# hjr37/diff-gaussian-rasterization

Hardware: AMD Instinct MI355X
Metric: Mviews/sec fwd+bwd @1080p, 500k Gaussians (higher is better)
Workload: dtype f32

## Files before the change

diff-gaussian-rasterization_amd/csrc/render_common.h:

```cpp
#pragma once
#include "dgr_common.h"
#include "kernels.h"
#include "wave_reduce.h"
#include "exact_math.h"

namespace dgr {

__device__ __forceinline__ uint4 blend_slot(const uint4* __restrict__ sched, const uint2* __restrict__ ranges,
                                            const uint32_t* __restrict__ sched_flag, int tiles, bool* overflowed = nullptr,
                                            bool* quadrant_lists = nullptr) {
    const int flag = __builtin_amdgcn_readfirstlane((int)*sched_flag);
    if (overflowed) *overflowed = (flag & 2) != 0;
    if (quadrant_lists) *quadrant_lists = (flag & 4) != 0;
    if (flag & 1) return sched[blockIdx.x];
    const int tile = xcd_contiguous((int)blockIdx.x, tiles);
    const uint2 r = ranges[tile];
    return make_uint4((uint32_t)tile, r.x, r.y, 0u);
}

__device__ __forceinline__ bool wave_any(bool p) { return __builtin_amdgcn_ballot_w64(p) != 0ull; }

namespace {

constexpr float LOG2E = 1.4426950408889634f, LN2 = 0.6931471805599453f;
constexpr float ALPHA_MIN = 15.0f / 255.0f;

enum { ALPHA_REF = 0, ALPHA_FAST = 1, ALPHA_GLIBC = 2 };
template <int AM>
struct AlphaPath {
    static constexpr bool LOG2 = (AM == ALPHA_FAST);
    static constexpr float PSCALE = LOG2 ? LOG2E : 1.0f;
    static constexpr float PUNSCALE = LOG2 ? LN2 : 1.0f;
    static constexpr bool TABLE = (AM == ALPHA_GLIBC);
};
template <int AM, bool UNTESTED_ARG = false>
__device__ __forceinline__ float alpha_raw(float o, float p2, const uint64_t* tab) {
    if (AM == ALPHA_FAST) return o * __builtin_amdgcn_exp2f(p2);
    if (AM == ALPHA_GLIBC) return o * exp_glibc<UNTESTED_ARG>(p2, tab);
    return o * exp_p32<UNTESTED_ARG>(p2);
}
template <int AM>
__device__ __forceinline__ float t_div(float T, float om, float& inv) {
    if (AM == ALPHA_FAST) { inv = __builtin_amdgcn_rcpf(om); return T * inv; }
    return div_ref(T, om, inv);
}

template <int NB, typename LIST_T = unsigned short, int NLISTS = 4, bool KEEP_ID = true>
struct StagedT {
    typedef LIST_T list_t;
    static constexpr bool HAS_ID = KEEP_ID;
    static constexpr int SLOTS = NB;
    static constexpr int SENTINEL = NB;
    static constexpr int LIST_LD = NB + 8;
    float4 rec[2 * (NB + 1)];
    float4 rgbd[NB + 1];
    uint32_t id[KEEP_ID ? NB : 1];
    LIST_T list[NLISTS][LIST_LD];
    int cnt4[4][NLISTS];
};
using Staged = StagedT<DGR_TILE_PIX>;

template <bool HALF_CODES>
__device__ __forceinline__ unsigned reach_code(const float4& q0, const float4& q1, float l2, float tile_x0, float tile_y0);

template <int AM, bool HALF_CODES = false, class S>
__device__ __forceinline__ unsigned stage_one(S& s, int slot, uint32_t gid, const float4* __restrict__ rec,
                                              float tile_x0, float tile_y0) {
    const float4 q0 = rec[DGR_REC_STRIDE * (size_t)gid + 0];
    const float4 q1 = rec[DGR_REC_STRIDE * (size_t)gid + 1];
    const float4 q2 = rec[DGR_REC_STRIDE * (size_t)gid + 2];
    const float o = q0.w;
    const float l2 = __log2f(o * (255.0f / 15.0f));
    constexpr float PSCALE = AlphaPath<AM>::PSCALE;
    float lthr = (o > 0.f) ? (-l2 * (AlphaPath<AM>::LOG2 ? 1.0f : LN2) - 1.0e-4f) : 3.0e38f;
    float zword = __int_as_float(slot);
    if (HALF_CODES) {
        lthr = fmaxf(lthr, -3.0e38f);
        lthr = __int_as_float(((__float_as_int(lthr) + 0xFF) & ~0xFF) | slot);
        zword = 0.f;
    }
    s.rec[2 * slot] = make_float4(q0.x, q0.y, -0.5f * PSCALE * q1.x, -0.5f * PSCALE * q1.z);
    s.rec[2 * slot + 1] = make_float4(-PSCALE * q1.y, o, zword, lthr);
    s.rgbd[slot] = make_float4(q2.x, q2.y, q2.z, q0.z);
    if (S::HAS_ID) s.id[slot] = gid;
    return reach_code<HALF_CODES>(q0, q1, l2, tile_x0, tile_y0);
}
template <bool HALF_CODES>
__device__ __forceinline__ unsigned reach_code(const float4& q0, const float4& q1, float l2, float tile_x0, float tile_y0) {
    const float tau = 2.0f * 0.6931471805599453f * l2;
    const float det = q1.x * q1.z - q1.y * q1.y;
    if (!(tau > 0.0f)) return 0u;
    if (!(det > 0.0f && q1.x > 0.0f && q1.z > 0.0f)) return HALF_CODES ? 0xFFu : 0xFu;
    const float k = tau * __builtin_amdgcn_rcpf(det);
    const float hx = __builtin_amdgcn_sqrtf(k * q1.z) * 1.001f + 0.05f, hy = __builtin_amdgcn_sqrtf(k * q1.x) * 1.001f + 0.05f;
    const float gx = q0.x - tile_x0, gy = q0.y - tile_y0;
    const bool xl = (gx + hx >= 0.0f) && (gx - hx <= 7.0f), xr = (gx + hx >= 8.0f) && (gx - hx <= 15.0f);
    if (HALF_CODES) {
        const float lo = gy - hy, hi = gy + hy;
        const unsigned xm = (xl ? 0x33u : 0u) | (xr ? 0xCCu : 0u);
        const unsigned ym = ((hi >= 0.0f) && (lo <= 3.0f) ? 0x05u : 0u) | ((hi >= 4.0f) && (lo <= 7.0f) ? 0x0Au : 0u) |
                            ((hi >= 8.0f) && (lo <= 11.0f) ? 0x50u : 0u) | ((hi >= 12.0f) && (lo <= 15.0f) ? 0xA0u : 0u);
        return xm & ym;
    }
    const bool yt = (gy + hy >= 0.0f) && (gy - hy <= 7.0f), yb = (gy + hy >= 8.0f) && (gy - hy <= 15.0f);
    return (xl && yt ? 1u : 0u) | (xr && yt ? 2u : 0u) | (xl && yb ? 4u : 0u) | (xr && yb ? 8u : 0u);
}

constexpr int TAG_SHIFT = DGR_TAG_SHIFT;
constexpr uint32_t ID_MASK = DGR_ID_MASK;
enum { TAGS_BYTES_QUADRANT = 1, TAGS_BYTES_HALVES = 2 };

__device__ __forceinline__ uint8_t* half_tags(const uint32_t* point_list, const uint32_t* sched_flag) {
    return carve_binning(reinterpret_cast<char*>(const_cast<uint32_t*>(point_list)), (size_t)sched_flag[-1]).pair_cov;
}
__device__ __forceinline__ uint32_t spread4(uint32_t c) { return (c & 1u) | ((c & 2u) << 1) | ((c & 4u) << 2) | ((c & 8u) << 3); }
__device__ __forceinline__ uint32_t fold8(uint32_t t) {
    t = (t | (t >> 1)) & 0x55u;
    return (t & 1u) | ((t >> 1) & 2u) | ((t >> 2) & 4u) | ((t >> 3) & 8u);
}

__device__ __forceinline__ uint32_t pack4(uint32_t w) { return (w & 1u) | ((w >> 7) & 2u) | ((w >> 14) & 4u) | ((w >> 21) & 8u); }
__device__ __forceinline__ uint32_t tag_byte(uint32_t up, uint32_t lo) { return spread4(pack4(up)) | (spread4(pack4(lo)) << 1); }

template <int AM, int TAGS, class S>
__device__ __forceinline__ unsigned stage_tagged(S& s, int slot, uint32_t entry, const float4* __restrict__ rec,
                                                 const uint8_t* __restrict__ tag8) {
    constexpr float PSCALE = AlphaPath<AM>::PSCALE;
    unsigned code = (unsigned)*tag8;
    if (code == 0u) return 0u;
    if (TAGS == TAGS_BYTES_QUADRANT) code = fold8(code);
    const uint32_t gid = entry & ID_MASK;
    const float4 q0 = rec[DGR_REC_STRIDE * (size_t)gid + 0];
    const float4 q1 = rec[DGR_REC_STRIDE * (size_t)gid + 1];
    const float4 q2 = rec[DGR_REC_STRIDE * (size_t)gid + 2];
    s.rec[2 * slot] = make_float4(q0.x, q0.y, -0.5f * PSCALE * q1.x, -0.5f * PSCALE * q1.z);
    s.rec[2 * slot + 1] = make_float4(-PSCALE * q1.y, q0.w, __int_as_float(slot * 4), __int_as_float(slot * 16));
    s.rgbd[slot] = make_float4(q2.x, q2.y, q2.z, q0.z);
    s.id[slot] = gid;
    return code;
}

__device__ __forceinline__ int lanes_below(unsigned long long m) {
    return (int)__builtin_amdgcn_mbcnt_hi((unsigned)(m >> 32), __builtin_amdgcn_mbcnt_lo((unsigned)m, 0u));
}

template <class S>
__device__ __forceinline__ int build_lists(S& s, unsigned code, int tid, int wave, int lane) {
    typedef typename S::list_t LT;
    unsigned long long bal[4];
#pragma unroll
    for (int w = 0; w < 4; w++) {
        bal[w] = __ballot((code >> w) & 1u);
        if (lane == 0) s.cnt4[wave][w] = __popcll(bal[w]);
    }
    __syncthreads();
#pragma unroll
    for (int w = 0; w < 4; w++) {
        if ((code >> w) & 1u) {
            int base = 0;
            for (int sw = 0; sw < wave; sw++) base += s.cnt4[sw][w];
            s.list[w][base + lanes_below(bal[w])] = (LT)(tid * 32);
        }
    }
    const int n = __builtin_amdgcn_readfirstlane(s.cnt4[0][wave] + s.cnt4[1][wave] + s.cnt4[2][wave] + s.cnt4[3][wave]);
    __syncthreads();
    if (lane < 4) s.list[wave][n + lane] = (LT)(S::SENTINEL * 32);
    return n;
}

template <class S>
__device__ __forceinline__ int build_half_lists(S& s, unsigned code, int tid, int wave, int lane) {
    typedef typename S::list_t LT;
    unsigned long long bal[8];
#pragma unroll
    for (int l = 0; l < 8; l++) {
        bal[l] = __ballot((code >> l) & 1u);
        if (lane == 0) s.cnt4[wave][l] = __popcll(bal[l]);
    }
    __syncthreads();
    int before = 0, all = 0;
    if (lane < 8) {
#pragma unroll
        for (int sw = 0; sw < 4; sw++) {
            const int c = s.cnt4[sw][lane];
            before += sw < wave ? c : 0;
            all += c;
        }
    }
#pragma unroll
    for (int l = 0; l < 8; l++) {
        const int base = __builtin_amdgcn_readlane(before, l);
        if ((code >> l) & 1u) s.list[l][base + lanes_below(bal[l])] = (LT)(tid * 32);
    }
    const int l0 = 2 * wave;
    const int n0 = __builtin_amdgcn_readlane(all, l0), n1 = __builtin_amdgcn_readlane(all, l0 + 1);
    __syncthreads();
    const int n = max(n0, n1);
    for (int i = n0 + lane; i < n + 4; i += 64) s.list[l0][i] = (LT)(S::SENTINEL * 32);
    for (int i = n1 + lane; i < n + 4; i += 64) s.list[l0 + 1][i] = (LT)(S::SENTINEL * 32);
    return n;
}

template <class S>
__device__ __forceinline__ int build_paired_lists(S& s, unsigned code8, int tid, int wave, int lane, unsigned long long (&split)[2]) {
    typedef typename S::list_t LT;
    static_assert(sizeof(LT) == 4 && S::SLOTS <= 128, "paired lists: 32-bit entries, at most two ranks per lane");
    unsigned long long bal[4];
#pragma unroll
    for (int w = 0; w < 4; w++) {
        bal[w] = __ballot(((code8 >> (2 * w)) & 3u) != 0u);
        if (lane == 0) s.cnt4[wave][w] = __popcll(bal[w]);
    }
    __syncthreads();
    int before = 0, all = 0;
    if (lane < 4) {
#pragma unroll
        for (int sw = 0; sw < 4; sw++) {
            const int c = s.cnt4[sw][lane];
            before += sw < wave ? c : 0;
            all += c;
        }
    }
#pragma unroll
    for (int w = 0; w < 4; w++) {
        const unsigned t = (code8 >> (2 * w)) & 3u;
        const int base = __builtin_amdgcn_readlane(before, w);
        if (t != 0u) s.list[2 * w][base + lanes_below(bal[w])] = (LT)(tid * 32) | t;
    }
    const int n = __builtin_amdgcn_readlane(all, wave);
    __syncthreads();
    LT* const LU = s.list[2 * wave];
    LT* const LL = s.list[2 * wave + 1];
    if (n <= 64) {
        const bool have = lane < n;
        const unsigned e0 = have ? LU[lane] : 0u;
        const int t0 = (int)(e0 & 3u);
        const int tm1 = __builtin_amdgcn_update_dpp(0, t0, 0x138, 0xf, 0xf, true);
        const int tm2 = __builtin_amdgcn_update_dpp(0, tm1, 0x138, 0xf, 0xf, true);
        const int tp1 = __builtin_amdgcn_update_dpp(0, t0, 0x130, 0xf, 0xf, true);
        const int tp2 = __builtin_amdgcn_update_dpp(0, tp1, 0x130, 0xf, 0xf, true);
        const bool odd = (lane & 1) != 0;
        const bool a_self = odd ? (tm1 * t0 == 2) : (t0 * tp1 == 2);
        const bool a_side = odd ? (tp1 * tp2 == 2) : (tm2 * tm1 == 2);
        const bool p2 = !a_self && !a_side && (odd ? (t0 * tp1 == 2) : (tm1 * t0 == 2));
        const bool first = odd ? p2 : a_self, second = odd ? a_self : p2;
        const unsigned long long keep = __ballot(have && !second);
        const int steps = __popcll(keep);
        if (have) {
            const int st = lanes_below(keep) - (second ? 1 : 0);
            const LT o = e0 & ~3u;
            if (first || second) {
                (t0 == 1 ? LU : LL)[st] = o;
            } else {
                LU[st] = o;
                LL[st] = o;
            }
        }
        if (lane < 4) {
            LU[steps + lane] = (LT)(S::SENTINEL * 32);
            LL[steps + lane] = (LT)(S::SENTINEL * 32);
        }
        split[0] = __ballot(lane < steps && LU[lane] != LL[lane]);
        split[1] = 0ull;
        return steps;
    }
    const LT ea = lane < n ? LU[lane] : 0u, eb = lane + 64 < n ? LU[lane + 64] : 0u;
    if (lane < n) { LU[lane] = ea & ~3u; LL[lane] = ea & ~3u; }
    if (lane + 64 < n) { LU[lane + 64] = eb & ~3u; LL[lane + 64] = eb & ~3u; }
    if (lane < 4) {
        LU[n + lane] = (LT)(S::SENTINEL * 32);
        LL[n + lane] = (LT)(S::SENTINEL * 32);
    }
    split[0] = split[1] = 0ull;
    return n;
}

typedef float f2 __attribute__((ext_vector_type(2)));

template <int AM>
__device__ __forceinline__ float pair_p2(const float4& q0, const float4& q1, f2 pxy, f2& dxy) {
    const f2 g = {q0.x, q0.y}, ac = {q0.z, q0.w};
    dxy = g - pxy;
    if (AM == ALPHA_FAST) {
        const f2 m = ac * dxy;
        const float t = __builtin_fmaf(q1.x, dxy.y, m.x);
        return __builtin_fmaf(dxy.x, t, m.y * dxy.y);
    } else {
#pragma clang fp contract(off)
        const f2 m = (ac * dxy) * dxy;
        const float B = (q1.x * dxy.x) * dxy.y;
        return (m.x + m.y) + B;
    }
}

template <class S>
__device__ __forceinline__ void load2(const S& s, int wave, int k, float4 (&q0)[2], float4 (&q1)[2]) {
    typedef typename S::list_t LT;
    unsigned off[2];
    if (sizeof(LT) == 4) {
        const uint2 pk = *reinterpret_cast<const uint2*>(&s.list[wave][k]);
        off[0] = pk.x;
        off[1] = pk.y;
    } else {
        const unsigned pk = *reinterpret_cast<const unsigned*>(&s.list[wave][k]);
        off[0] = pk & 0xffffu;
        off[1] = pk >> 16;
    }
    const char* base = reinterpret_cast<const char*>(s.rec);
#pragma unroll
    for (int u = 0; u < 2; u++) {
        q0[u] = *reinterpret_cast<const float4*>(base + off[u]);
        q1[u] = *reinterpret_cast<const float4*>(base + off[u] + 16);
    }
}


template <bool TAGGED = false, class S>
__device__ __forceinline__ void write_sentinel(S& s) {
    constexpr int NB = S::SLOTS;
    s.rec[2 * NB] = make_float4(0.f, 0.f, 0.f, 0.f);
    s.rec[2 * NB + 1] = make_float4(0.f, 0.f, __int_as_float(TAGGED ? NB * 4 : NB), TAGGED ? __int_as_float(NB * 16) : 3.0e38f);
    s.rgbd[NB] = make_float4(0.f, 0.f, 0.f, 0.f);
}

constexpr int NACC = DGR_ACC_STRIDE;
constexpr int ACC_LD = DGR_TILE_PIX + 1;

template <int NCOMP, int LD = ACC_LD>
__device__ __forceinline__ void flush_acc(const float* lds_acc, const uint32_t* ids, int cnt, float* global_acc, int tid) {
    const int comp = tid & 15;
    if (comp < NCOMP) {
        for (int r = tid >> 4; r < cnt; r += 16) {
            const float v = lds_acc[comp * LD + r];
            if (v != 0.f) atomicAdd(global_acc + (size_t)ids[r] * DGR_ACC_STRIDE + comp, v);
        }
    }
}

}
}
```

diff-gaussian-rasterization_amd/csrc/render_light.hip:

```cpp
#include "render_common.h"

namespace dgr {
namespace {

constexpr int FWD_UNROLL = 2;

template <bool HALVES>
struct StagedFwd {
    typedef StagedT<DGR_TILE_PIX, unsigned short, HALVES ? 8 : 4, !HALVES> staged_t;
    staged_t f;
    float unc[DGR_TILE_PIX];
    uint32_t cnt[DGR_TILE_PIX];
    uint32_t hit[DGR_TILE_PIX];
    uint64_t exptab[32];
};


template <class SF>
__device__ __forceinline__ void flush_slot(const SF& sf, const RenderFwdLightArgs& a, uint8_t* tag8, uint32_t pos0, int tid, bool staged) {
    if (!staged) return;
    uint32_t t8;
    if constexpr (!SF::staged_t::HAS_ID) {
        t8 = tag_byte(sf.hit[tid], __float_as_uint(sf.f.rec[2 * tid + 1].z));
    } else {
        t8 = spread4(pack4(sf.hit[tid])) * 3u;
    }
    tag8[pos0 + tid] = (uint8_t)t8;
    if (sf.cnt[tid] != 0u) {
        uint32_t gid;
        if constexpr (SF::staged_t::HAS_ID) gid = sf.f.id[tid];
        else gid = a.point_list[pos0 + tid];
        atomicAdd(&a.gau_uncertainty[gid], sf.unc[tid]);
        atomicAdd(&a.gau_related_pixels[gid], (int)sf.cnt[tid]);
    }
}

template <int AM, bool HALVES>
__device__ __forceinline__ void render_fwd_light_body(const RenderFwdLightArgs& a, StagedFwd<HALVES>& sf, const uint4 slot, const bool overflowed) {
    typename StagedFwd<HALVES>::staged_t& s = sf.f;
    const int tile = (int)slot.x;
    const int tx = tile % a.grid_x, ty = tile / a.grid_x;
    const int tid = threadIdx.x, wave = tid >> 6, lane = tid & 63;
    const int px = tx * DGR_BLOCK_X + (wave & 1) * 8 + (lane & 7);
    const int py = ty * DGR_BLOCK_Y + (wave >> 1) * 8 + (lane >> 3);
    const bool inside = px < a.W && py < a.H;
    const uint32_t pix_id = (uint32_t)a.W * (uint32_t)py + (uint32_t)px;
    const f2 pxy = {(float)px, (float)py};
    const float tile_x0 = (float)(tx * DGR_BLOCK_X), tile_y0 = (float)(ty * DGR_BLOCK_Y);
    const int my_list = HALVES ? 2 * wave + (lane >> 5) : wave;
    uint8_t* const tag8 = half_tags(a.point_list, a.sched_flag);
    unsigned char* const mark_base = (HALVES && lane >= 32) ? reinterpret_cast<unsigned char*>(&s.rec[1].z) + wave
                                                             : reinterpret_cast<unsigned char*>(sf.hit) + wave;
    const int mark_stride = (HALVES && lane >= 32) ? 32 : 4;

    const uint2 range = make_uint2(slot.y, slot.z);
    const int total = (int)(range.y - range.x);

    float T = 1.0f, C0 = 0.f, C1 = 0.f, C2 = 0.f, weight = 0.f, Dd = 0.f, D_median = 0.f;
    uint32_t last_contributor = 0;
    float ub = inside ? 0.f : -__builtin_inff();
    const float gt_px = inside ? a.gt_depth[pix_id] : 0.f;
    if (tid == 0) write_sentinel(s);
    if (AlphaPath<AM>::TABLE) exp_ref_table_fill(sf.exptab, tid);
    bool have_flush = false;
    int last_base = 0;

    for (int base = 0; base < total; base += DGR_TILE_PIX) {
        if (__syncthreads_and(ub < 0.f)) break;
        last_base = base;
        if (have_flush) flush_slot(sf, a, tag8, range.x + base - DGR_TILE_PIX, tid, true);
        sf.unc[tid] = 0.f;
        sf.cnt[tid] = 0u;
        sf.hit[tid] = 0u;
        have_flush = true;
        const int cnt = min(DGR_TILE_PIX, total - base);
        unsigned code = 0;
        if (tid < cnt) code = stage_one<AM, HALVES>(s, tid, a.point_list[range.x + base + tid], a.rec, tile_x0, tile_y0);
        const int n = HALVES ? build_half_lists(s, code, tid, wave, lane) : build_lists(s, code, tid, wave, lane);

        for (int k = 0; k < n; k += FWD_UNROLL) {
            float4 q0[FWD_UNROLL], q1[FWD_UNROLL];
            load2(s, my_list, k, q0, q1);
#pragma unroll
            for (int u = 0; u < FWD_UNROLL; u++) {
                f2 dxy;
                const float p2 = pair_p2<AM>(q0[u], q1[u], pxy, dxy);
                if ((p2 <= ub) & (p2 >= q1[u].w)) {
                  const float alpha = fminf(0.99f, alpha_raw<AM>(q1[u].y, p2, sf.exptab));
                  if (alpha >= ALPHA_MIN) {
#pragma clang fp contract(off)
                    const float test_T = T * (1.0f - alpha);
                    if (test_T < 0.0001f) {
                        ub = -__builtin_inff();
                    } else {
                        const int j = HALVES ? (__float_as_int(q1[u].w) & 0xFF) : __float_as_int(q1[u].z);
                        const float4 cd = s.rgbd[j];
                        mark_base[j * mark_stride] = 1;
                        const float w = alpha * T;
                        C0 = __builtin_fmaf(cd.x, w, C0); C1 = __builtin_fmaf(cd.y, w, C1); C2 = __builtin_fmaf(cd.z, w, C2);
                        weight = weight + w;
                        Dd = __builtin_fmaf(cd.w, w, Dd);
                        if (T > 0.5f && test_T < 0.5f) {
                            D_median = cd.w;
                            const float e = cd.w - gt_px;
                            atomicAdd(&sf.unc[j], e * e * w);
                            atomicAdd(&sf.cnt[j], 1u);
                        }
                        T = test_T;
                        last_contributor = (uint32_t)(base + j + 1);
                    }
                  }
                }
            }
            if (!wave_any(ub >= 0.f)) break;
        }
    }
    __syncthreads();
    if (have_flush) flush_slot(sf, a, tag8, range.x + last_base, tid, tid < total - last_base);
    for (int p = (have_flush ? last_base + DGR_TILE_PIX : 0) + tid; p < total; p += DGR_TILE_PIX) tag8[range.x + p] = 0;

    if (overflowed) {
        C0 = C1 = C2 = weight = Dd = D_median = __builtin_nanf("");
    }
    if (inside) {
        const uint32_t N = (uint32_t)a.W * (uint32_t)a.H;
        a.n_contrib[pix_id] = last_contributor;
        a.out_color[pix_id] = C0 + T * a.bg[0];
        a.out_color[N + pix_id] = C1 + T * a.bg[1];
        a.out_color[2 * N + pix_id] = C2 + T * a.bg[2];
        a.out_alpha[pix_id] = weight;
        a.out_depth[pix_id] = Dd;
        a.out_median[pix_id] = D_median;
        a.out_depth_var[pix_id] = 0.0f;
    }
}

template <int AM>
__global__ void __launch_bounds__(256, 8) render_fwd_light_kernel(RenderFwdLightArgs a) {
    __shared__ union { StagedFwd<true> h; StagedFwd<false> q; } sf;
    if (a.rep.host && blockIdx.x == 0 && threadIdx.x == 0) report_status(a.rep, a.status);
    bool overflowed, quadrant_lists;
    const uint4 slot = blend_slot(a.sched, a.ranges, a.sched_flag, a.grid_x * a.grid_y, &overflowed, &quadrant_lists);
    if (quadrant_lists) render_fwd_light_body<AM, false>(a, sf.q, slot, overflowed);
    else render_fwd_light_body<AM, true>(a, sf.h, slot, overflowed);
}

constexpr int NACC_LIGHT = 14;

template <bool DET, bool HALVES = false, bool ABS = false>
struct StagedBwd {
    static constexpr int NB = DET ? 64 : 128;
    static constexpr int LD = NB + 1;
    static constexpr int PLANE = NACC_LIGHT * LD;
    static constexpr int NACC = ABS ? NACC_LIGHT + 2 : NACC_LIGHT;
    typedef StagedT<NB, uint32_t, HALVES ? 8 : 4> staged_t;
    staged_t f;
    float acc[(DET ? 4 : 1) * PLANE + (ABS ? 2 * LD : 0)];
    uint32_t inst[DET ? NB : 1];
    int max_last;
    uint64_t exptab[32];
};

template <int AM, bool DO_MAP, bool DO_POSE, bool DET, bool LEAN, bool HALVES, bool ABS = false>
__device__ __forceinline__ void render_bwd_light_body(const RenderBwdLightArgs& a, StagedBwd<DET, HALVES, ABS>& sb, const uint4 slot,
                                                      float* __restrict__ abs_out = nullptr) {
    static_assert(!HALVES || !DET, "half-wave / paired lists: not with the deterministic kernel's planes (LDS)");
    static_assert(!ABS || (DO_MAP && !DET), "absgrad: the mapping backward, not the deterministic kernel");
    constexpr bool PAIRED = HALVES && DO_MAP;
    typedef StagedBwd<DET, HALVES, ABS> SB;
    constexpr int BWD_NB = SB::NB, BWD_LD = SB::LD;
    typename SB::staged_t& s = sb.f;
    const int tile = (int)slot.x;
    const int tx = tile % a.grid_x, ty = tile / a.grid_x;
    const int tid = threadIdx.x, wave = tid >> 6, lane = tid & 63;
    const int px = tx * DGR_BLOCK_X + (wave & 1) * 8 + (lane & 7);
    const int py = ty * DGR_BLOCK_Y + (wave >> 1) * 8 + (lane >> 3);
    const bool inside = px < a.W && py < a.H;
    const uint32_t pix_id = (uint32_t)a.W * (uint32_t)py + (uint32_t)px;
    const uint32_t N = (uint32_t)a.W * (uint32_t)a.H;
    const float pxf = (float)px, pyf = (float)py;
    const f2 pxy = {pxf, pyf};

    const uint2 range = make_uint2(slot.y, slot.z);
    const int last_contributor = inside ? (int)a.n_contrib[pix_id] : 0;

    if (tid == 0) {
        sb.max_last = 0;
        write_sentinel<true>(s);
    }
    if (AlphaPath<AM>::TABLE) exp_ref_table_fill(sb.exptab, tid);
    __syncthreads();
    {
        int v = last_contributor;
#pragma unroll
        for (int off = 32; off > 0; off >>= 1) v = max(v, __shfl_xor(v, off, 64));
        if (lane == 0) atomicMax(&sb.max_last, v);
    }
    __syncthreads();
    const int total = min((int)(range.y - range.x), sb.max_last);
    if (total <= 0) return;

    const float T_final = inside ? (1.0f - a.alphas[pix_id]) : 0.f;
    float T = T_final;
    float dpix0 = 0.f, dpix1 = 0.f, dpix2 = 0.f, dpix_depth = 0.f, dpix_median = 0.f, dpix_var = 0.f, gt_px = 0.f;
    if (inside) {
        dpix0 = __builtin_nontemporal_load(a.dL_dpix + pix_id);
        dpix1 = __builtin_nontemporal_load(a.dL_dpix + N + pix_id);
        dpix2 = __builtin_nontemporal_load(a.dL_dpix + 2 * N + pix_id);
        dpix_depth = __builtin_nontemporal_load(a.dL_dpix_depth + pix_id);
        if (!LEAN) {
            if (a.dL_dpix_median) dpix_median = __builtin_nontemporal_load(a.dL_dpix_median + pix_id);
            if (a.dL_dpix_var) dpix_var = __builtin_nontemporal_load(a.dL_dpix_var + pix_id);
            gt_px = __builtin_nontemporal_load(a.gt_depth + pix_id);
        }
    }
    const float bg_term = -T_final * (a.bg[0] * dpix0 + a.bg[1] * dpix1 + a.bg[2] * dpix2);
    const float ddelx_dx = 0.5f * a.W, ddely_dy = 0.5f * a.H;
    float S = 0.f;
    float mid_thr = 0.5f;
    int my_comp;
    if (DO_MAP) {
        const int c = (lane >= 48) ? 12 : wave_reduce12d_comp(lane);
        my_comp = ((lane & 3) != 0 || c > 11) ? -1 : (c == 10 ? (DO_POSE ? 13 : 10) : c == 11 ? (DO_POSE ? 10 : -1) : c);
    } else if (HALVES) {
        const int c = half_reduce3_comp(lane);
        my_comp = c == 0 ? 4 : c == 1 ? 5 : c == 2 ? 13 : -1;
    } else {
        const int c = wave_reduce4_comp(lane);
        my_comp = ((lane & 15) == 0 && c < 3) ? (c == 0 ? 4 : c == 1 ? 5 : 13) : -1;
    }
    const int my_list = HALVES ? 2 * wave + (lane >> 5) : wave;
    const uint8_t* const tag8 = half_tags(a.point_list, a.sched_flag);

    float* const my_acc = sb.acc + (DET ? wave * SB::PLANE : 0) + (my_comp >= 0 ? my_comp : 0) * BWD_LD;

    for (int hi = total; hi > 0; hi -= BWD_NB) {
        const int lo = max(0, hi - BWD_NB);
        const int cnt = hi - lo;
        __syncthreads();
        unsigned code = 0;
        if (tid < cnt) code = stage_tagged<AM, HALVES ? TAGS_BYTES_HALVES : TAGS_BYTES_QUADRANT>(s, tid, a.point_list[range.x + lo + tid], a.rec, tag8 + (range.x + lo + tid));
        if (!DET) {
#pragma unroll
            for (int k = 0; k < SB::NACC; k++)
                if (BWD_NB == DGR_TILE_PIX || tid < BWD_NB) sb.acc[k * BWD_LD + tid] = 0.f;
        }
        unsigned long long split[2] = {0ull, 0ull};
        const int n = PAIRED   ? build_paired_lists(s, code, tid, wave, lane, split)
                      : HALVES ? build_half_lists(s, code, tid, wave, lane)
                               : build_lists(s, code, tid, wave, lane);
        const int rel_last4 = 4 * (last_contributor - lo);

        constexpr int U = PAIRED ? 1 : 2;
        for (int k = ((n + U - 1) / U) * U - U; k >= 0; k -= U) {
            float4 q0[2], q1[2];
            if (U == 2) {
                load2(s, my_list, k, q0, q1);
            } else {
                const unsigned off = s.list[my_list][k];
                q0[0] = *reinterpret_cast<const float4*>(reinterpret_cast<const char*>(s.rec) + off);
                q1[0] = *reinterpret_cast<const float4*>(reinterpret_cast<const char*>(s.rec) + off + 16);
            }
#pragma unroll
            for (int u = U - 1; u >= 0; u--) {
                f2 dxy;
                const float p2 = pair_p2<AM>(q0[u], q1[u], pxy, dxy);
                const float dx = dxy.x, dy = dxy.y;
                const int j4 = __float_as_int(q1[u].z);
                const float oG = alpha_raw<AM, true>(q1[u].y, p2, sb.exptab);
                const bool valid = (j4 < rel_last4) & (p2 <= 0.0f) & !(oG < ALPHA_MIN);
                const float oGm = valid ? oG : 0.f;
                const float alpha = fminf(0.99f, oGm);
                const float4 cd = *reinterpret_cast<const float4*>(reinterpret_cast<const char*>(s.rgbd) + __float_as_int(q1[u].w));
                const float om = 1.f - alpha;
                float inv;
                T = t_div<AM>(T, om, inv);
                const float w = alpha * T;
                const float e = cd.w - gt_px;
                const float X = LEAN ? cd.x * dpix0 + cd.y * dpix1 + cd.z * dpix2 + cd.w * dpix_depth
                                     : cd.x * dpix0 + cd.y * dpix1 + cd.z * dpix2 + cd.w * dpix_depth + (e * e) * dpix_var;
                const float dL_dalpha = (X - S) * T + bg_term * inv;
                S = alpha * X + om * S;
                const float qq = oGm * dL_dalpha;
                const float qdx = qq * dx, qdy = qq * dy;
                const float wd = w * dpix_depth;
                float tot;
                if (DO_MAP) {
                    float gmed = 0.f;
                    if (!LEAN) {
                        const bool fire = valid & (T > mid_thr);
                        gmed = fire ? dpix_median : 0.f;
                        mid_thr = fire ? __builtin_inff() : mid_thr;
                    }
                    float g[12];
                    g[0] = w * dpix0;
                    g[1] = w * dpix1;
                    g[2] = w * dpix2;
                    g[3] = LEAN ? wd : wd + 2.f * ((dpix_var * w) * e);
                    g[4] = qdx;
                    g[5] = qdy;
                    g[6] = qdx * dx;
                    g[7] = qdx * dy;
                    g[8] = qdy * dy;
                    g[9] = qq;
                    g[10] = DO_POSE ? wd : gmed;
                    g[11] = DO_POSE ? gmed : 0.f;
                    if (ABS) {
                        constexpr float UN = AlphaPath<AM>::PUNSCALE;
                        const float ca = q0[u].z * (-2.f * UN), cb = q1[u].x * (-UN), cc = q0[u].w * (-2.f * UN);
                        const float h = half_reduce3(fabsf(ca * qdx + cb * qdy), fabsf(cc * qdy + cb * qdx), 0.f);
                        const int c = half_reduce3_comp(lane);
                        if (c == 0 || c == 1)
                            atomicAdd(reinterpret_cast<float*>(reinterpret_cast<char*>(sb.acc) + j4 + (NACC_LIGHT + c) * (BWD_LD * 4)), h);
                    }
                    if (PAIRED) {
                        float u0, u1;
                        wave_reduce12d_head(g, u0, u1);
                        const int st = k + u;
                        if ((split[st >> 6] >> (st & 63)) & 1ull) {
                            const float r0 = quad_sum(u0), r1 = quad_sum(u1);
                            auto comp_of = [](int slot) { return slot < 10 ? slot : slot == 10 ? (DO_POSE ? 13 : 10) : (DO_POSE ? 10 : -1); };
                            const int s1 = wave_reduce12d_half_slot1(lane);
                            const int c0 = (lane & 3) == 0 ? comp_of(wave_reduce12d_half_slot0(lane)) : -1;
                            const int c1 = ((lane & 3) == 0 && s1 >= 0) ? comp_of(s1) : -1;
                            char* const col = reinterpret_cast<char*>(sb.acc) + j4;
                            if (c0 >= 0) atomicAdd(reinterpret_cast<float*>(col + c0 * (BWD_LD * 4)), r0);
                            if (c1 >= 0) atomicAdd(reinterpret_cast<float*>(col + c1 * (BWD_LD * 4)), r1);
                            continue;
                        }
                        tot = wave_reduce12d_tail(u0, u1);
                    } else {
                        tot = wave_reduce12d(g);
                    }
                } else if (HALVES) {
                    tot = half_reduce3(qdx, qdy, wd);
                } else {
                    float g4[4] = {qdx, qdy, wd, 0.f};
                    tot = wave_reduce4(g4);
                }
                if (my_comp >= 0) {
                    float* const cell = reinterpret_cast<float*>(reinterpret_cast<char*>(my_acc) + j4);
                    if (DET) *cell = tot; else atomicAdd(cell, tot);
                }
            }
        }

        __syncthreads();
        if (DET && tid < BWD_NB) {
            uint32_t row = ~0u;
            if (code != 0u) {
#pragma unroll
                for (int k = 0; k < NACC_LIGHT; k++) {
                    const bool delivered = DO_MAP ? (k <= 9 || k == 10 || (DO_POSE && k == 13)) : (k == 4 || k == 5 || k == 13);
                    float v = 0.f;
                    if (delivered) {
#pragma unroll
                        for (int w = 0; w < 4; w++)
                            if ((code >> w) & 1u) v += sb.acc[w * SB::PLANE + k * BWD_LD + tid];
                    }
                    sb.acc[k * BWD_LD + tid] = v;
                }
                const uint32_t gid = s.id[tid];
                const ushort4 rc = a.det_rect[gid];
                row = a.det_goff[gid] + (uint32_t)(ty - (int)rc.y) * (uint32_t)(rc.z - rc.x) + (uint32_t)(tx - (int)rc.x);
            }
            sb.inst[tid] = row;
        }
        if (DET) __syncthreads();
        if (code != 0u) {
            constexpr float UN = AlphaPath<AM>::PUNSCALE;
            const float4 r0 = s.rec[2 * tid], r1 = s.rec[2 * tid + 1];
            const float ca = r0.z * (-2.f * UN), cb = r1.x * (-UN), cc = r0.w * (-2.f * UN);
            const float Sx = sb.acc[4 * BWD_LD + tid], Sy = sb.acc[5 * BWD_LD + tid];
            sb.acc[4 * BWD_LD + tid] = -(ca * Sx + cb * Sy) * ddelx_dx;
            sb.acc[5 * BWD_LD + tid] = -(cc * Sy + cb * Sx) * ddely_dy;
            if (ABS) {
                const float ax = sb.acc[NACC_LIGHT * BWD_LD + tid] * ddelx_dx, ay = sb.acc[(NACC_LIGHT + 1) * BWD_LD + tid] * ddely_dy;
                const size_t gid = s.id[tid];
                if (ax != 0.f) atomicAdd(abs_out + 3 * gid, ax);
                if (ay != 0.f) atomicAdd(abs_out + 3 * gid + 1, ay);
            }
            if (DO_MAP) {
                sb.acc[6 * BWD_LD + tid] *= -0.5f;
                sb.acc[7 * BWD_LD + tid] *= -0.5f;
                sb.acc[8 * BWD_LD + tid] *= -0.5f;
                sb.acc[9 * BWD_LD + tid] *= __builtin_amdgcn_rcpf(r1.y);
            }
        }
        __syncthreads();
        if (DET) {
            const int comp = tid & 15;
            for (int r = tid >> 4; r < cnt; r += 16) {
                const uint32_t row = sb.inst[r];
                if (row < a.det_R && comp < NACC_LIGHT) a.det_rows[(size_t)row * DGR_ACC_STRIDE + comp] = sb.acc[comp * BWD_LD + r];
            }
        } else {
            flush_acc<NACC_LIGHT, BWD_LD>(sb.acc, s.id, cnt, a.acc, tid);
        }
    }
}

template <int AM, bool DO_POSE, bool LEAN, bool BY_FRAME>
__global__ void __launch_bounds__(256, LEAN ? 8 : 7) render_bwd_light_abs_kernel(RenderBwdLightArgs a, float* abs_out) {
    __shared__ union { StagedBwd<false, BY_FRAME, true> h; StagedBwd<false, false, true> q; } sb;
    bool quadrant_lists = true;
    const uint4 slot = blend_slot(a.sched, a.ranges, a.sched_flag, a.grid_x * a.grid_y, nullptr, BY_FRAME ? &quadrant_lists : nullptr);
    if (BY_FRAME && !quadrant_lists) render_bwd_light_body<AM, true, DO_POSE, false, LEAN, BY_FRAME, true>(a, sb.h, slot, abs_out);
    else render_bwd_light_body<AM, true, DO_POSE, false, LEAN, false, true>(a, sb.q, slot, abs_out);
}

template <int AM, bool DO_MAP, bool DO_POSE, bool DET = false, bool LEAN = false, bool BY_FRAME = false>
__global__ void __launch_bounds__(256, 8) render_bwd_light_kernel(RenderBwdLightArgs a) {
    static_assert(!BY_FRAME || !DET, "the deterministic kernel walks quadrant lists");
    __shared__ union { StagedBwd<DET, BY_FRAME> h; StagedBwd<DET, false> q; } sb;
    bool quadrant_lists = true;
    const uint4 slot = blend_slot(a.sched, a.ranges, a.sched_flag, a.grid_x * a.grid_y, nullptr, BY_FRAME ? &quadrant_lists : nullptr);
    if (BY_FRAME && !quadrant_lists) render_bwd_light_body<AM, DO_MAP, DO_POSE, DET, LEAN, BY_FRAME>(a, sb.h, slot);
    else render_bwd_light_body<AM, DO_MAP, DO_POSE, DET, LEAN, false>(a, sb.q, slot);
}

__device__ __forceinline__ uint32_t rect_tiles(ushort4 r) { return (r.z > r.x && r.w > r.y) ? (uint32_t)(r.z - r.x) * (uint32_t)(r.w - r.y) : 0u; }
__global__ void __launch_bounds__(256) det_block_sums_kernel(int P, const ushort4* __restrict__ rect, uint32_t* __restrict__ blk) {
    __shared__ uint32_t red[4];
    const int g = blockIdx.x * 256 + threadIdx.x;
    uint32_t v = g < P ? rect_tiles(rect[g]) : 0u;
#pragma unroll
    for (int off = 32; off > 0; off >>= 1) v += __shfl_xor(v, off, 64);
    if ((threadIdx.x & 63) == 0) red[threadIdx.x >> 6] = v;
    __syncthreads();
    if (threadIdx.x == 0) blk[blockIdx.x] = red[0] + red[1] + red[2] + red[3];
}
__global__ void __launch_bounds__(256) det_offsets_kernel(int P, const ushort4* __restrict__ rect, const uint32_t* __restrict__ blk,
                                                          uint32_t* __restrict__ goff) {
    __shared__ uint32_t red[4], wsum[4];
    uint32_t before = 0;
    for (int b = threadIdx.x; b < (int)blockIdx.x; b += 256) before += blk[b];
#pragma unroll
    for (int off = 32; off > 0; off >>= 1) before += __shfl_xor(before, off, 64);
    if ((threadIdx.x & 63) == 0) red[threadIdx.x >> 6] = before;
    const int g = blockIdx.x * 256 + threadIdx.x;
    const uint32_t n = g < P ? rect_tiles(rect[g]) : 0u;
    uint32_t incl = n;
#pragma unroll
    for (int off = 1; off < 64; off <<= 1) {
        const uint32_t v = __shfl_up(incl, off, 64);
        if ((threadIdx.x & 63) >= off) incl += v;
    }
    if ((threadIdx.x & 63) == 63) wsum[threadIdx.x >> 6] = incl;
    __syncthreads();
    uint32_t base = red[0] + red[1] + red[2] + red[3];
    for (int w = 0; w < (int)(threadIdx.x >> 6); w++) base += wsum[w];
    if (g < P) goff[g] = base + incl - n;
}
__global__ void __launch_bounds__(256) det_gather_kernel(int P, const ushort4* __restrict__ rect, const uint32_t* __restrict__ goff,
                                                         const float* __restrict__ rows, uint32_t R, float* __restrict__ acc) {
    const int g = blockIdx.x * 16 + (threadIdx.x >> 4), comp = threadIdx.x & 15;
    if (g >= P) return;
    uint32_t n = rect_tiles(rect[g]);
    if (n == 0u) return;
    const uint32_t first = goff[g];
    if (first >= R || n > R - first) {
        acc[(size_t)g * DGR_ACC_STRIDE + comp] = __builtin_nanf("");
        return;
    }
    const float* r = rows + (size_t)first * DGR_ACC_STRIDE + comp;
    float v = 0.f;
    for (uint32_t i = 0; i < n; i++) v += r[(size_t)i * DGR_ACC_STRIDE];
    acc[(size_t)g * DGR_ACC_STRIDE + comp] = v;
}

__global__ void __launch_bounds__(64) wave_reduce_test_kernel(const float* in, float* out16, float* out12, float* out4,
                                                             int* comp16, int* comp12, int* comp4) {
    const int lane = threadIdx.x;
    float g16[16], g12[12], g4[4];
#pragma unroll
    for (int k = 0; k < 16; k++) g16[k] = in[k * 64 + lane];
#pragma unroll
    for (int k = 0; k < 12; k++) g12[k] = g16[k];
#pragma unroll
    for (int k = 0; k < 4; k++) g4[k] = g16[k];
    out16[lane] = wave_reduce16d(g16);
    out12[lane] = wave_reduce12d(g12);
    out4[lane] = wave_reduce4(g4);
    comp16[lane] = wave_reduce16d_comp(lane);
    comp12[lane] = wave_reduce12d_comp(lane);
    comp4[lane] = wave_reduce4_comp(lane);
}

__global__ void __launch_bounds__(64) half_reduce_test_kernel(const float* in, float* r0, float* r1, float* h3, int* slot0, int* slot1,
                                                             int* comp3) {
    const int lane = threadIdx.x;
    float g[12];
#pragma unroll
    for (int k = 0; k < 12; k++) g[k] = in[k * 64 + lane];
    h3[lane] = half_reduce3(g[0], g[1], g[2]);
    float u0, u1;
    wave_reduce12d_head(g, u0, u1);
    r0[lane] = quad_sum(u0);
    r1[lane] = quad_sum(u1);
    slot0[lane] = wave_reduce12d_half_slot0(lane);
    slot1[lane] = wave_reduce12d_half_slot1(lane);
    comp3[lane] = half_reduce3_comp(lane);
}

__global__ void __launch_bounds__(64) half_reduce16_test_kernel(const float* in, float* r0, float* r1, int* slot0, int* slot1) {
    const int lane = threadIdx.x;
    float g[16];
#pragma unroll
    for (int k = 0; k < 16; k++) g[k] = in[k * 64 + lane];
    float u0, u1;
    wave_reduce16d_head(g, u0, u1);
    r0[lane] = quad_sum(u0);
    r1[lane] = quad_sum(u1);
    slot0[lane] = wave_reduce16d_half_slot0(lane);
    slot1[lane] = wave_reduce16d_half_slot1(lane);
}

__global__ void __launch_bounds__(256) lane_lists_test_kernel(const unsigned char* codes, uint32_t* paired, uint32_t* halves) {
    typedef StagedT<128, uint32_t, 8> S;
    __shared__ S s;
    const int tid = threadIdx.x, wave = tid >> 6, lane = tid & 63;
    const unsigned code = tid < 128 ? codes[tid] : 0u;
    for (int pass = 0; pass < 2; pass++) {
        for (int i = tid; i < 8 * S::LIST_LD; i += 256) (&s.list[0][0])[i] = 0xFFFFFFFFu;
        __syncthreads();
        unsigned long long split[2] = {0ull, 0ull};
        const int n = pass == 0 ? build_paired_lists(s, code, tid, wave, lane, split) : build_half_lists(s, code, tid, wave, lane);
        uint32_t* const o = (pass == 0 ? paired : halves) + 280 * wave;
        if (lane == 0) {
            o[0] = (uint32_t)n;
            o[1] = (uint32_t)split[0]; o[2] = (uint32_t)(split[0] >> 32);
            o[3] = (uint32_t)split[1]; o[4] = (uint32_t)(split[1] >> 32);
        }
        for (int i = lane; i < S::LIST_LD; i += 64) {
            o[5 + i] = s.list[2 * wave][i];
            o[5 + S::LIST_LD + i] = s.list[2 * wave + 1][i];
        }
        __syncthreads();
    }
}

template <bool GLIBC>
__global__ void __launch_bounds__(256) exact_math_test_kernel(int n, const float* x, const float* a, const float* b, float* out_exp,
                                                             float* out_div) {
    __shared__ uint64_t tab[32];
    exp_ref_table_fill(tab, threadIdx.x);
    __syncthreads();
    for (int i = blockIdx.x * 256 + threadIdx.x; i < n; i += gridDim.x * 256) {
        out_exp[i] = GLIBC ? exp_glibc<true>(x[i], tab) : exp_p32<true>(x[i]);
        float inv;
        out_div[i] = t_div<ALPHA_REF>(a[i], b[i], inv);
    }
}

template <int AM>
void launch_bwd_light_mode(const RenderBwdLightArgs& a, int tiles, hipStream_t stream) {
    if (AM == ALPHA_REF && !a.det_rows && !a.dL_dpix_median && !a.dL_dpix_var) {
        if (!a.map_off && !a.track_off)
            launch_blend((render_bwd_light_kernel<ALPHA_REF, true, true, false, true, true>), dim3(tiles), dim3(256), stream, a);
        else if (!a.map_off)
            launch_blend((render_bwd_light_kernel<ALPHA_REF, true, false, false, true, true>), dim3(tiles), dim3(256), stream, a);
        else
            launch_blend((render_bwd_light_kernel<ALPHA_REF, false, true, false, true, true>), dim3(tiles), dim3(256), stream, a);
        return;
    }
    if (AM == ALPHA_REF && a.det_rows) {
        if (!a.map_off && !a.track_off)
            launch_blend((render_bwd_light_kernel<ALPHA_REF, true, true, true>), dim3(tiles), dim3(256), stream, a);
        else if (!a.map_off)
            launch_blend((render_bwd_light_kernel<ALPHA_REF, true, false, true>), dim3(tiles), dim3(256), stream, a);
        else
            launch_blend((render_bwd_light_kernel<ALPHA_REF, false, true, true>), dim3(tiles), dim3(256), stream, a);
        return;
    }
    constexpr bool BF = AM != ALPHA_GLIBC;
    if (!a.map_off && !a.track_off)
        launch_blend((render_bwd_light_kernel<AM, true, true, false, false, BF>), dim3(tiles), dim3(256), stream, a);
    else if (!a.map_off)
        launch_blend((render_bwd_light_kernel<AM, true, false, false, false, BF>), dim3(tiles), dim3(256), stream, a);
    else
        launch_blend((render_bwd_light_kernel<AM, false, true, false, false, BF>), dim3(tiles), dim3(256), stream, a);
}
}

hipError_t launch_render_fwd_light(const RenderFwdLightArgs& a, int alpha_mode, hipStream_t stream) {
    const int tiles = a.grid_x * a.grid_y;
    if (tiles <= 0) return hipSuccess;
    switch (alpha_mode) {
        case ALPHA_FAST: launch_blend(render_fwd_light_kernel<ALPHA_FAST>, dim3(tiles), dim3(256), stream, a); break;
        case ALPHA_GLIBC: launch_blend(render_fwd_light_kernel<ALPHA_GLIBC>, dim3(tiles), dim3(256), stream, a); break;
        default: launch_blend(render_fwd_light_kernel<ALPHA_REF>, dim3(tiles), dim3(256), stream, a);
    }
    return hipGetLastError();
}
hipError_t launch_render_bwd_light(const RenderBwdLightArgs& a, int alpha_mode, hipStream_t stream) {
    const int tiles = a.grid_x * a.grid_y;
    if (tiles <= 0 || (a.track_off && a.map_off)) return hipSuccess;
    switch (alpha_mode) {
        case ALPHA_FAST: launch_bwd_light_mode<ALPHA_FAST>(a, tiles, stream); break;
        case ALPHA_GLIBC: launch_bwd_light_mode<ALPHA_GLIBC>(a, tiles, stream); break;
        default: launch_bwd_light_mode<ALPHA_REF>(a, tiles, stream);
    }
    return hipGetLastError();
}
hipError_t launch_render_bwd_light_abs(const RenderBwdLightArgs& a, float* dL_dmean2D_abs, int alpha_mode, hipStream_t stream) {
    const int tiles = a.grid_x * a.grid_y;
    if (tiles <= 0 || a.map_off) return hipSuccess;
    const bool lean = !a.dL_dpix_median && !a.dL_dpix_var;
    if (alpha_mode == ALPHA_FAST) {
        if (!a.track_off) launch_blend((render_bwd_light_abs_kernel<ALPHA_FAST, true, false, true>), dim3(tiles), dim3(256), stream, a, dL_dmean2D_abs);
        else launch_blend((render_bwd_light_abs_kernel<ALPHA_FAST, false, false, true>), dim3(tiles), dim3(256), stream, a, dL_dmean2D_abs);
    } else if (alpha_mode == ALPHA_REF && lean) {
        if (!a.track_off) launch_blend((render_bwd_light_abs_kernel<ALPHA_REF, true, true, true>), dim3(tiles), dim3(256), stream, a, dL_dmean2D_abs);
        else launch_blend((render_bwd_light_abs_kernel<ALPHA_REF, false, true, true>), dim3(tiles), dim3(256), stream, a, dL_dmean2D_abs);
    } else if (alpha_mode == ALPHA_REF) {
        if (!a.track_off) launch_blend((render_bwd_light_abs_kernel<ALPHA_REF, true, false, true>), dim3(tiles), dim3(256), stream, a, dL_dmean2D_abs);
        else launch_blend((render_bwd_light_abs_kernel<ALPHA_REF, false, false, true>), dim3(tiles), dim3(256), stream, a, dL_dmean2D_abs);
    } else {
        return hipErrorInvalidValue;
    }
    return hipGetLastError();
}
namespace {
__global__ void __launch_bounds__(256) zero_floats_kernel(float* dst, size_t n) {
    const size_t stride = (size_t)gridDim.x * 256;
    for (size_t i = (size_t)blockIdx.x * 256 + threadIdx.x; i < n; i += stride) dst[i] = 0.f;
}
}
hipError_t launch_zero_floats(float* dst, size_t n, hipStream_t stream) {
    if (n == 0) return hipSuccess;
    const unsigned blocks = (unsigned)std::min<size_t>((n + 255) / 256, 256 * 16);
    launch(zero_floats_kernel, dim3(blocks), dim3(256), stream, dst, n);
    return hipGetLastError();
}
hipError_t launch_det_offsets(int P, const ushort4* rect, uint32_t* blk, uint32_t* goff, hipStream_t stream) {
    if (P <= 0) return hipSuccess;
    const int nb = (P + 255) / 256;
    launch(det_block_sums_kernel, dim3(nb), dim3(256), stream, P, rect, blk);
    launch(det_offsets_kernel, dim3(nb), dim3(256), stream, P, rect, (const uint32_t*)blk, goff);
    return hipGetLastError();
}
hipError_t launch_det_gather(int P, const ushort4* rect, const uint32_t* goff, const float* rows, uint32_t R, float* acc, hipStream_t stream) {
    if (P <= 0) return hipSuccess;
    launch(det_gather_kernel, dim3((P + 15) / 16), dim3(256), stream, P, rect, goff, rows, R, acc);
    return hipGetLastError();
}
hipError_t launch_exact_math_test(int n, const float* x, const float* a, const float* b, float* out_exp, float* out_div,
                                  int alpha_mode, hipStream_t stream) {
    if (n <= 0) return hipSuccess;
    if (alpha_mode == ALPHA_GLIBC)
        launch(exact_math_test_kernel<true>, dim3(min((n + 255) / 256, 4096)), dim3(256), stream, n, x, a, b, out_exp, out_div);
    else
        launch(exact_math_test_kernel<false>, dim3(min((n + 255) / 256, 4096)), dim3(256), stream, n, x, a, b, out_exp, out_div);
    return hipGetLastError();
}
hipError_t launch_wave_reduce_test(const float* in, float* out16, float* out12, float* out4, int* comp16, int* comp12, int* comp4,
                                   hipStream_t stream) {
    launch(wave_reduce_test_kernel, dim3(1), dim3(64), stream, in, out16, out12, out4, comp16, comp12, comp4);
    return hipGetLastError();
}

hipError_t launch_half_reduce_test(const float* in, float* r0, float* r1, float* h3, int* slot0, int* slot1, int* comp3, hipStream_t stream) {
    launch(half_reduce_test_kernel, dim3(1), dim3(64), stream, in, r0, r1, h3, slot0, slot1, comp3);
    return hipGetLastError();
}
hipError_t launch_half_reduce16_test(const float* in, float* r0, float* r1, int* slot0, int* slot1, hipStream_t stream) {
    launch(half_reduce16_test_kernel, dim3(1), dim3(64), stream, in, r0, r1, slot0, slot1);
    return hipGetLastError();
}
hipError_t launch_lane_lists_test(const unsigned char* codes, uint32_t* paired, uint32_t* halves, hipStream_t stream) {
    launch(lane_lists_test_kernel, dim3(1), dim3(256), stream, codes, paired, halves);
    return hipGetLastError();
}

}
```

Measured before the change: 0.002600.

## Compact tagged entries into backward batches, skipping untagged list positions

```diff
diff --git a/diff-gaussian-rasterization_amd/csrc/render_common.h b/diff-gaussian-rasterization_amd/csrc/render_common.h
--- a/diff-gaussian-rasterization_amd/csrc/render_common.h
+++ b/diff-gaussian-rasterization_amd/csrc/render_common.h
@@ -123,10 +123,8 @@
 __device__ __forceinline__ uint32_t tag_byte(uint32_t up, uint32_t lo) { return spread4(pack4(up)) | (spread4(pack4(lo)) << 1); }
 
 template <int AM, int TAGS, class S>
-__device__ __forceinline__ unsigned stage_tagged(S& s, int slot, uint32_t entry, const float4* __restrict__ rec,
-                                                 const uint8_t* __restrict__ tag8) {
+__device__ __forceinline__ unsigned stage_tag_byte(S& s, int slot, uint32_t entry, const float4* __restrict__ rec, unsigned code) {
     constexpr float PSCALE = AlphaPath<AM>::PSCALE;
-    unsigned code = (unsigned)*tag8;
     if (code == 0u) return 0u;
     if (TAGS == TAGS_BYTES_QUADRANT) code = fold8(code);
     const uint32_t gid = entry & ID_MASK;
@@ -138,6 +136,11 @@
     s.rgbd[slot] = make_float4(q2.x, q2.y, q2.z, q0.z);
     s.id[slot] = gid;
     return code;
+}
+template <int AM, int TAGS, class S>
+__device__ __forceinline__ unsigned stage_tagged(S& s, int slot, uint32_t entry, const float4* __restrict__ rec,
+                                                 const uint8_t* __restrict__ tag8) {
+    return stage_tag_byte<AM, TAGS>(s, slot, entry, rec, (unsigned)*tag8);
 }
 
 __device__ __forceinline__ int lanes_below(unsigned long long m) {
@@ -326,16 +329,18 @@
 constexpr int NACC = DGR_ACC_STRIDE;
 constexpr int ACC_LD = DGR_TILE_PIX + 1;
 
-template <int NCOMP, int LD = ACC_LD>
+template <int NCOMP, int LD = ACC_LD, bool LOCAL_ADDR = false>
 __device__ __forceinline__ void flush_acc(const float* lds_acc, const uint32_t* ids, int cnt, float* global_acc, int tid) {
     const int comp = tid & 15;
     if (comp < NCOMP) {
         for (int r = tid >> 4; r < cnt; r += 16) {
             const float v = lds_acc[comp * LD + r];
-            if (v != 0.f) atomicAdd(global_acc + (size_t)ids[r] * DGR_ACC_STRIDE + comp, v);
-        }
-    }
-}
-
-}
-}
+            int c = comp;
+            if (LOCAL_ADDR) asm volatile("" : "+v"(c));
+            if (v != 0.f) atomicAdd(global_acc + (size_t)ids[r] * DGR_ACC_STRIDE + c, v);
+        }
+    }
+}
+
+}
+}
diff --git a/diff-gaussian-rasterization_amd/csrc/render_light.hip b/diff-gaussian-rasterization_amd/csrc/render_light.hip
--- a/diff-gaussian-rasterization_amd/csrc/render_light.hip
+++ b/diff-gaussian-rasterization_amd/csrc/render_light.hip
@@ -157,6 +157,10 @@
     staged_t f;
     float acc[(DET ? 4 : 1) * PLANE + (ABS ? 2 * LD : 0)];
     uint32_t inst[DET ? NB : 1];
+    int pos[NB];
+    uint8_t code[DET ? NB : 1];
+    alignas(16) int wcnt[4];
+    int next_hi;
     int max_last;
     uint64_t exptab[32];
 };
@@ -234,22 +238,53 @@
 
     float* const my_acc = sb.acc + (DET ? wave * SB::PLANE : 0) + (my_comp >= 0 ? my_comp : 0) * BWD_LD;
 
-    for (int hi = total; hi > 0; hi -= BWD_NB) {
-        const int lo = max(0, hi - BWD_NB);
-        const int cnt = hi - lo;
+    for (int hi = total; hi > 0;) {
+        constexpr int WIN = DGR_TILE_PIX;
+        const int p = hi - WIN + tid;
+        unsigned t8 = 0u;
+        uint32_t entry = 0u;
+        if (p >= 0) {
+            t8 = tag8[range.x + p];
+            entry = a.point_list[range.x + p];
+        }
+        const unsigned long long bt = __ballot(t8 != 0u);
         __syncthreads();
+        if (lane == 0) sb.wcnt[wave] = __popcll(bt);
+        __syncthreads();
+        const int4 wc = *reinterpret_cast<const int4*>(sb.wcnt);
+        const int ntag = __builtin_amdgcn_readfirstlane(wc.x + wc.y + wc.z + wc.w);
+        if (ntag == 0) {
+            hi -= WIN;
+            continue;
+        }
+        const int cnt = min(ntag, BWD_NB);
+        const int above = __popcll((bt >> lane) >> 1) + (wave < 1 ? wc.y : 0) + (wave < 2 ? wc.z : 0) + (wave < 3 ? wc.w : 0);
         unsigned code = 0;
-        if (tid < cnt) code = stage_tagged<AM, HALVES ? TAGS_BYTES_HALVES : TAGS_BYTES_QUADRANT>(s, tid, a.point_list[range.x + lo + tid], a.rec, tag8 + (range.x + lo + tid));
+        int slot = 0;
+        if (t8 != 0u && above < BWD_NB) {
+            slot = cnt - 1 - above;
+            code = stage_tag_byte<AM, HALVES ? TAGS_BYTES_HALVES : TAGS_BYTES_QUADRANT>(s, slot, entry, a.rec, t8);
+            sb.pos[slot] = p;
+            if (DET) sb.code[slot] = (uint8_t)code;
+            if (above == BWD_NB - 1) sb.next_hi = p;
+        }
         if (!DET) {
 #pragma unroll
             for (int k = 0; k < SB::NACC; k++)
                 if (BWD_NB == DGR_TILE_PIX || tid < BWD_NB) sb.acc[k * BWD_LD + tid] = 0.f;
         }
         unsigned long long split[2] = {0ull, 0ull};
-        const int n = PAIRED   ? build_paired_lists(s, code, tid, wave, lane, split)
-                      : HALVES ? build_half_lists(s, code, tid, wave, lane)
-                               : build_lists(s, code, tid, wave, lane);
-        const int rel_last4 = 4 * (last_contributor - lo);
+        const int n = PAIRED   ? build_paired_lists(s, code, slot, wave, lane, split)
+                      : HALVES ? build_half_lists(s, code, slot, wave, lane)
+                               : build_lists(s, code, slot, wave, lane);
+        int nv = cnt;
+        if (wave_any(last_contributor < hi)) {
+            nv = 0;
+#pragma unroll
+            for (int step = BWD_NB; step > 0; step >>= 1)
+                if (nv + step <= cnt && sb.pos[nv + step - 1] < last_contributor) nv += step;
+        }
+        const int rel_last4 = 4 * nv;
 
         constexpr int U = PAIRED ? 1 : 2;
         for (int k = ((n + U - 1) / U) * U - U; k >= 0; k -= U) {
@@ -348,6 +383,7 @@
         __syncthreads();
         if (DET && tid < BWD_NB) {
             uint32_t row = ~0u;
+            const unsigned code = tid < cnt ? sb.code[tid] : 0u;
             if (code != 0u) {
 #pragma unroll
                 for (int k = 0; k < NACC_LIGHT; k++) {
@@ -367,7 +403,7 @@
             sb.inst[tid] = row;
         }
         if (DET) __syncthreads();
-        if (code != 0u) {
+        if (tid < cnt) {
             constexpr float UN = AlphaPath<AM>::PUNSCALE;
             const float4 r0 = s.rec[2 * tid], r1 = s.rec[2 * tid + 1];
             const float ca = r0.z * (-2.f * UN), cb = r1.x * (-UN), cc = r0.w * (-2.f * UN);
@@ -395,8 +431,9 @@
                 if (row < a.det_R && comp < NACC_LIGHT) a.det_rows[(size_t)row * DGR_ACC_STRIDE + comp] = sb.acc[comp * BWD_LD + r];
             }
         } else {
-            flush_acc<NACC_LIGHT, BWD_LD>(sb.acc, s.id, cnt, a.acc, tid);
-        }
+            flush_acc<NACC_LIGHT, BWD_LD, !DO_MAP>(sb.acc, s.id, cnt, a.acc, tid);
+        }
+        hi = cnt == BWD_NB ? __builtin_amdgcn_readfirstlane(sb.next_hi) : hi - WIN;
     }
 }
 
diff --git a/profiles/kernel_resources.py b/profiles/kernel_resources.py
--- /dev/null
+++ b/profiles/kernel_resources.py
@@ -0,0 +1,17 @@
+import re,sys,subprocess
+def res(path):
+    txt=open(path).read()
+    out={}
+    for blk in re.split(r"\n  - ", txt.split("amdhsa.kernels:")[1]):
+        name=re.search(r"\.name:\s+(\S+)",blk)
+        if not name: continue
+        n=name.group(1)
+        if "bwd_light" not in n: continue
+        g=lambda k: (re.search(r"\."+k+r":\s+(\d+)",blk) or [None,"?"])[1]
+        dem=subprocess.run(["c++filt",n],capture_output=True,text=True).stdout.strip()
+        dem=dem.replace("dgr::(anonymous namespace)::","").replace("(dgr::RenderBwdLightArgs)","").replace("(dgr::RenderBwdLightArgs, float*)","")
+        out[dem]=(g("vgpr_count"),g("agpr_count"),g("group_segment_fixed_size"),g("private_segment_fixed_size"),g("vgpr_spill_count"))
+    return out
+a=res(sys.argv[1]); b=res(sys.argv[2])
+print("%-70s %s"%("kernel","vgpr agpr lds scratch spill : base -> new"))
+for k in a: print("%-70s %s -> %s"%(k,a[k],b.get(k)))
diff --git a/profiles/tag_account.py b/profiles/tag_account.py
--- /dev/null
+++ b/profiles/tag_account.py
@@ -0,0 +1,142 @@
+#!/usr/bin/env python3
+import argparse
+import json
+import os
+import sys
+
+ROOT = os.path.dirname(os.path.dirname(os.path.abspath(__file__)))
+PKG = os.path.join(ROOT, "diff-gaussian-rasterization_amd")
+for p in (ROOT, PKG, os.path.join(PKG, "light"), os.path.join(ROOT, "tests")):
+    if p not in sys.path:
+        sys.path.insert(0, p)
+
+import numpy as np
+
+
+def batches(tagged, nb, window):
+    total = len(tagged)
+    pos = np.flatnonzero(tagged)
+    plain = []
+    for hi in range(total, 0, -nb):
+        lo = max(0, hi - nb)
+        plain.append(pos[np.searchsorted(pos, lo):np.searchsorted(pos, hi)])
+    comp, empty = [], 0
+    hi = total
+    while hi > 0:
+        lo = max(0, hi - window)
+        a, b = np.searchsorted(pos, lo), np.searchsorted(pos, hi)
+        n = b - a
+        if n == 0:
+            empty += 1
+            hi = lo
+            continue
+        comp.append(pos[max(a, b - nb):b])
+        hi = int(pos[b - nb]) if n >= nb else lo
+    return plain, comp, empty
+
+
+def paired_steps(types):
+    n = len(types)
+    if n == 0:
+        return 0
+    if n > 64:
+        return n
+    t = np.zeros(n + 4, np.int64)
+    t[2:n + 2] = types
+    t0, tm1, tm2, tp1, tp2 = t[2:n + 2], t[1:n + 1], t[0:n], t[3:n + 3], t[4:n + 4]
+    odd = (np.arange(n) & 1) == 1
+    a_self = np.where(odd, tm1 * t0 == 2, t0 * tp1 == 2)
+    a_side = np.where(odd, tp1 * tp2 == 2, tm2 * tm1 == 2)
+    p2 = ~a_self & ~a_side & np.where(odd, t0 * tp1 == 2, tm1 * t0 == 2)
+    second = np.where(odd, a_self, p2)
+    return int(np.count_nonzero(~second))
+
+
+def list_stats(bl, tag8):
+    entries = steps = 0
+    for b in bl:
+        tb = tag8[b].astype(np.int64)
+        for w in range(4):
+            ty = (tb >> (2 * w)) & 3
+            ty = ty[ty != 0]
+            entries += len(ty)
+            steps += paired_steps(ty)
+    return entries, steps
+
+
+def export_half_tags(hh, s, d):
+    import torch
+    from dgr_amd import _capi
+    lib = _capi.load()
+    R = d["num_rendered"]
+    dst = torch.zeros(max(R, 1), dtype=torch.uint8, device="cuda")
+    got = lib.dgr_state_export(_capi.stream_handle(), b"half_tags", s.P, s.W, s.H, R, hh.binning_capacity(d, s.W, s.H),
+                               _capi.ptr(d["geom"]), _capi.ptr(d["binning"]), _capi.ptr(d["img"]), dst.data_ptr())
+    assert got >= 0, _capi.last_error()
+    torch.cuda.synchronize()
+    return dst[:R].cpu().numpy()
+
+
+def main():
+    ap = argparse.ArgumentParser()
+    ap.add_argument("--P", type=int, default=500_000)
+    ap.add_argument("--W", type=int, default=1920)
+    ap.add_argument("--H", type=int, default=1080)
+    ap.add_argument("--scale", type=float, default=1.0)
+    ap.add_argument("--seed", type=int, default=0)
+    args = ap.parse_args()
+    from dgr_amd.synth import make_scene
+    import hip_helpers as hh
+    s = make_scene(args.P, args.W, args.H, seed=args.seed, view_index=0)
+    out, d = hh.hip_forward(s, 3, scale_modifier=args.scale)
+    ranges = hh.hip_state("ranges", s, d).reshape(-1, 2).astype(np.int64)
+    tags = export_half_tags(hh, s, d)
+    nc = hh.hip_state("n_contrib", s, d).astype(np.int64).reshape(args.H, args.W)
+    gx, gy = (args.W + 15) // 16, (args.H + 15) // 16
+    pad = np.zeros((gy * 16, gx * 16), np.int64)
+    pad[:args.H, :args.W] = nc
+    last = pad.reshape(gy, 16, gx, 16).max(axis=(1, 3)).reshape(-1)
+    res = {"P": args.P, "W": args.W, "H": args.H, "R": int(d["num_rendered"])}
+    for nb, window, key in ((128, 256, "nb128"), (64, 256, "nb64_det")):
+        below = tagged_n = plain = comp = empty = 0
+        full = 0
+        ls = {"positions": [0, 0], "tagged": [0, 0]}
+        per_tile = []
+        for t in range(len(ranges)):
+            a, b = ranges[t]
+            total = int(min(b - a, last[t]))
+            if total <= 0:
+                per_tile.append(0)
+                continue
+            t8 = tags[a:a + total]
+            tg = t8 != 0
+            below += total
+            tagged_n += int(tg.sum())
+            per_tile.append(int(tg.sum()))
+            p, c, e = batches(tg, nb, window)
+            plain += len(p)
+            comp += len(c)
+            empty += e
+            full += sum(1 for x in c if len(x) == nb)
+            if nb == 128:
+                for k, bl in (("positions", p), ("tagged", c)):
+                    en, st = list_stats(bl, t8)
+                    ls[k][0] += en
+                    ls[k][1] += st
+        res[key] = {"positions_below_total": below, "untagged_fraction": 1.0 - tagged_n / max(below, 1),
+                    "batches_positions": plain, "batches_tagged": comp, "full_batches_tagged": full, "empty_windows": empty,
+                    "batch_reduction": 1.0 - comp / max(plain, 1)}
+        if nb == 128:
+            res[key]["paired_lists"] = {k: {"quadrant_entries": v[0], "steps": v[1], "steps_per_entry": v[1] / max(v[0], 1),
+                                            "entries_per_quadrant_list": v[0] / max(4 * (plain if k == "positions" else comp), 1)}
+                                        for k, v in ls.items()}
+            pt = np.array(per_tile)
+            edges = [0, 1, 64, 128, 256, 512, 1024, 2048, 4096, 1 << 30]
+            h, _ = np.histogram(pt, bins=edges)
+            res["tagged_per_tile_hist"] = {f"[{edges[i]},{edges[i + 1]})": int(h[i]) for i in range(len(h))}
+            res["tagged_per_tile_mean"] = float(pt.mean())
+    print(json.dumps(res, indent=1))
+
+
+if __name__ == "__main__":
+    main()
```

Measured after the change: 0.002661, median of 6. 1.02x the previous value.
